# MOj0/vpt

Measured on AMD Instinct MI355X. Metric: volume samples/s, MCM 512^3 @ 1920x1080, higher is better.
Workload: dtype f32

## Files before the change

### vpt_amd/csrc/vpt_core.hip

```cpp
#include <chrono>
#include <memory>
#include "vpt_internal.h"
#include "vpt_kernels_layout.h"
#include "vpt_srgb_lut.h"

static thread_local char g_err[512] = "";
char *vpt_error_buffer(void) { return g_err; }
int fail(int code, const char *fmt, ...) {
    va_list ap; va_start(ap, fmt);
    vsnprintf(g_err, sizeof(g_err), fmt, ap);
    va_end(ap);
    return code;
}
extern "C" const char *vpt_last_error(void) { return g_err; }
extern "C" const char *vpt_version(void) { return "vpt-mi355x 0.1 (gfx950)"; }

extern "C" int vpt_device_count(int *count) {
    if (!count) return fail(VPT_ERR_INVALID, "count is null");
    HIP_TRY(hipGetDeviceCount(count));
    return VPT_OK;
}
extern "C" int vpt_context_create(int device, vpt_context **out) {
    if (!out) return fail(VPT_ERR_INVALID, "out is null");
    int n = 0;
// ... 940 lines not shown
static int profile_sum(const EventPairs &pairs, double *total_ms, uint32_t *launches) {
    double sum = 0.0; uint32_t n = 0;
    for (const EventPairs::Pair *p = pairs.first(); p; p = pairs.after(p)) {
        float ms = 0.0f;
        HIP_TRY(hipEventElapsedTime(&ms, p->t0, p->t1));
        sum += (double)ms; n += p->launches;
    }
    *total_ms = sum; *launches = n;
    return VPT_OK;
}
extern "C" int vpt_renderer_profile_side(vpt_renderer *r, double *total_ms, uint32_t *launches) {
    if (!r || !total_ms || !launches) return fail(VPT_ERR_INVALID, "null argument");
    HIP_TRY(hipSetDevice(r->ctx->device));
    VPT_TRY(join_side(r));
    HIP_TRY(hipStreamSynchronize(r->ctx->stream));
    return profile_sum(r->side_timing, total_ms, launches);
}
extern "C" int vpt_renderer_profile(vpt_renderer *r, double *total_ms, uint32_t *launches) {
    if (!r || !total_ms || !launches) return fail(VPT_ERR_INVALID, "null argument");
    HIP_TRY(hipSetDevice(r->ctx->device));
    HIP_TRY(hipStreamSynchronize(r->ctx->stream));
    return profile_sum(r->timing, total_ms, launches);
}

extern "C" int vpt_probe_math(vpt_context *c, int which, const float *in, float *out, size_t n) {
    if (!c || !in || !out) return fail(VPT_ERR_INVALID, "null argument");
    if (which < 0 || which > VPT_PROBE_POW) return fail(VPT_ERR_INVALID, "unknown probe %d", which);
    if (n == 0) return VPT_OK;
    HIP_TRY(hipSetDevice(c->device));
    size_t nin = (which == VPT_PROBE_ATAN2 || which == VPT_PROBE_MIN || which == VPT_PROBE_MAX || which == VPT_PROBE_POW) ? 2 * n : n;
    DevBuf<float> din, dout;
    HIP_TRY(din.alloc(nin));
    HIP_TRY(dout.alloc(n));
    HIP_TRY(hipMemcpyAsync(din, in, nin * sizeof(float), hipMemcpyHostToDevice, c->stream));
    hipLaunchKernelGGL(k_probe_math, dim3((unsigned)((n + 255) / 256)), dim3(256), 0, c->stream, which, din.get(), dout.get(), n);
    HIP_TRY(hipGetLastError());
    HIP_TRY(hipMemcpyAsync(out, dout, n * sizeof(float), hipMemcpyDeviceToHost, c->stream));
    HIP_TRY(hipStreamSynchronize(c->stream));
    return VPT_OK;
}
static int probe_sample(vpt_renderer *r, const float *xyz, float *rgba, size_t n, bool boundary) {
    if (!r || !xyz || !rgba) return fail(VPT_ERR_INVALID, "null argument");
    if (n == 0) return VPT_OK;
    vpt_context *c = r->ctx;
    HIP_TRY(hipSetDevice(c->device));
    PassArgs a;
    VPT_TRY(make_args(r, nullptr, true, &a));
    if (boundary && !a.vol.atlas) return fail(VPT_ERR_UNSUPPORTED, "the volume's boundary atlas is not in use (switched off, or a float volume with non-finite texels)");
    DevBuf<float> din; DevBuf<float4> dout;
    HIP_TRY(din.alloc(3 * n));
    HIP_TRY(dout.alloc(n));
    HIP_TRY(hipMemcpyAsync(din, xyz, 3 * n * sizeof(float), hipMemcpyHostToDevice, c->stream));
    dim3 grid((unsigned)((n + 255) / 256));
    const bool launched = dispatch_sampler_variant(variant_of(r), [&](auto V) {
        if (boundary) hipLaunchKernelGGL(k_probe_sample_boundary<V()>, grid, dim3(VPT_BLOCK), lds_bytes(r), c->stream, a, din.get(), dout.get(), n);
        else hipLaunchKernelGGL(k_probe_sample<V()>, grid, dim3(VPT_BLOCK), lds_bytes(r), c->stream, a, din.get(), dout.get(), n);
        return true;
    }, [] { return false; });
    if (!launched) return fail(VPT_ERR_INVALID, "no probe kernel for variant %d", variant_of(r));
    HIP_TRY(hipGetLastError());
    HIP_TRY(hipMemcpyAsync(rgba, dout, n * sizeof(float4), hipMemcpyDeviceToHost, c->stream));
    HIP_TRY(hipStreamSynchronize(c->stream));
    return VPT_OK;
}

extern "C" int vpt_probe_environment_texels(vpt_renderer *r, float *rgba, size_t n) {
    if (!r || !rgba) return fail(VPT_ERR_INVALID, "null argument");
    const size_t texels = (size_t)r->env_w * r->env_h;
    if (n < texels) return fail(VPT_ERR_INVALID, "environment table holds %zu texels, room for %zu", texels, n);
    vpt_context *c = r->ctx;
    HIP_TRY(hipSetDevice(c->device));
    VPT_TRY(join_side(r));
    HIP_TRY(hipMemcpyAsync(rgba, r->env, texels * sizeof(float4), hipMemcpyDeviceToHost, c->stream));
    HIP_TRY(hipStreamSynchronize(c->stream));
    return VPT_OK;
}
extern "C" int vpt_probe_sample(vpt_renderer *r, const float *xyz, float *rgba, size_t n) { return probe_sample(r, xyz, rgba, n, false); }
extern "C" int vpt_probe_sample_boundary(vpt_renderer *r, const float *xyz, float *rgba, size_t n) { return probe_sample(r, xyz, rgba, n, true); }

extern "C" int vpt_probe_stream_read(vpt_context *c, size_t nbytes, int iterations, double *gb_per_s) {
    if (!c || !gb_per_s) return fail(VPT_ERR_INVALID, "null argument");
    if (nbytes < (1u << 20) || iterations < 1) return fail(VPT_ERR_INVALID, "need at least 1 MiB and one iteration");
    HIP_TRY(hipSetDevice(c->device));
    size_t n16 = nbytes / 16;
    DevBuf<uint4> buf; DevBuf<uint32_t> sink;
    HIP_TRY(buf.alloc(n16));
    HIP_TRY(sink.alloc(1));
    HIP_TRY(hipMemsetAsync(buf, 0, n16 * 16, c->stream));
    Event e0, e1;
    float ms = 0.0f;
    HIP_TRY(e0.create());
    HIP_TRY(e1.create());
    dim3 grid(256 * 16);
    hipLaunchKernelGGL(k_stream_read, grid, dim3(VPT_BLOCK), 0, c->stream, buf.get(), n16, sink.get());
    HIP_TRY(hipEventRecord(e0, c->stream));
    for (int i = 0; i < iterations; i++) {
        hipLaunchKernelGGL(k_stream_read, grid, dim3(VPT_BLOCK), 0, c->stream, buf.get(), n16, sink.get());
        HIP_TRY(hipGetLastError());
    }
    HIP_TRY(hipEventRecord(e1, c->stream));
    HIP_TRY(hipEventSynchronize(e1));
    HIP_TRY(hipEventElapsedTime(&ms, e0, e1));
    *gb_per_s = (double)(n16 * 16) * iterations / ((double)ms * 1e-3) / 1e9;
    return VPT_OK;
}
```

### vpt_amd/csrc/vpt_device.h

```cpp
#pragma once
#include <hip/hip_runtime.h>
#include <stdint.h>
#include "vpt_variants.h"

#define VPT_DEV __device__ __forceinline__

struct f3 { float x, y, z; };
struct f2 { float x, y; };

VPT_DEV float vmin(float a, float b) { return fminf(a, b); }
VPT_DEV float vmax(float a, float b) { return fmaxf(a, b); }
VPT_DEV float vclamp01(float x) { return vmin(vmax(x, 0.0f), 1.0f); }
VPT_DEV float mixf(float a, float b, float t) { return fmaf(b, t, a * (1.0f - t)); }
VPT_DEV f3 mix3(f3 a, f3 b, float t) { return f3{ mixf(a.x, b.x, t), mixf(a.y, b.y, t), mixf(a.z, b.z, t) }; }
VPT_DEV float dot3(f3 a, f3 b) { return fmaf(a.z, b.z, fmaf(a.y, b.y, a.x * b.x)); }
VPT_DEV float length3(f3 a) { return sqrtf(dot3(a, a)); }
VPT_DEV f3 sub3(f3 a, f3 b) { return f3{ a.x - b.x, a.y - b.y, a.z - b.z }; }
VPT_DEV f3 madd3(f3 p, float t, f3 d) { return f3{ fmaf(t, d.x, p.x), fmaf(t, d.y, p.y), fmaf(t, d.z, p.z) }; }
VPT_DEV float lerpf(float a, float b, float f) { return fmaf(f, b - a, a); }
VPT_DEV float4 lerp4(float4 a, float4 b, float f) {
    return make_float4(lerpf(a.x, b.x, f), lerpf(a.y, b.y, f), lerpf(a.z, b.z, f), lerpf(a.w, b.w, f));
}

VPT_DEV float rcp_nr(float x) {
// ... 483 lines not shown
        uint32_t x, y, z; float fx, fy, fz;
        filter_cell<V>(p.x, v.fnx, v.hx, x, fx);
        filter_cell<V>(p.y, v.fny, v.hy, y, fy);
        filter_cell<V>(p.z, v.fnz, v.hz, z, fz);
        const float *b0 = (const float *)cell_addr<WIDE>(v, t, x, y, z);
        const bool lx = below_first(p.x, v.fnx), ly = below_first(p.y, v.fny), lz = below_first(p.z, v.fnz);
        f2 out = { 0.0f, 0.0f };
#pragma unroll
        for (int c = 0; c < (RG ? 2 : 1); c++) {
            const float *b = b0 + 128 * c;
            float2 r00, r10, r01, r11;
            __builtin_memcpy(&r00, b, 8); __builtin_memcpy(&r10, b + 5, 8); __builtin_memcpy(&r01, b + 25, 8); __builtin_memcpy(&r11, b + 30, 8);
            if (lx) { r00.y = r00.x; r10.y = r10.x; r01.y = r01.x; r11.y = r11.x; }
            if (ly) { r10 = r00; r11 = r01; }
            if (lz) { r01 = r00; r11 = r10; }
            float c00 = lerpf(r00.x, r00.y, fx), c10 = lerpf(r10.x, r10.y, fx);
            float c01 = lerpf(r01.x, r01.y, fx), c11 = lerpf(r11.x, r11.y, fx);
            const float val = lerpf(lerpf(c00, c10, fy), lerpf(c01, c11, fy), fz);
            if (c == 0) out.x = val; else out.y = val;
        }
        return out;
    }
    if (V & VPT_V_NEAREST) {
        uint32_t x = nearest_cell(p.x, v.fnx, v.hx), y = nearest_cell(p.y, v.fny, v.hy), z = nearest_cell(p.z, v.fnz, v.hz);
        const uint8_t *a = cell_addr<WIDE>(v, t, x, y, z);
        if (SNORM) return f2{ snorm_decode((float)(int8_t)a[0]), RG ? snorm_decode((float)(int8_t)a[128]) : 0.0f };
        return f2{ (float)a[0] * VPT_INV255, RG ? (float)a[128] * VPT_INV255 : 0.0f };
    }
    uint32_t x, y, z; float fx, fy, fz;
    filter_cell<V>(p.x, v.fnx, v.hx, x, fx);
    filter_cell<V>(p.y, v.fny, v.hy, y, fy);
    filter_cell<V>(p.z, v.fnz, v.hz, z, fz);
    if (V & VPT_V_REC) {
        const uint64_t w = record_load(record_addr<WIDE>(v, t, x, y, z));
        return f2{ record_blend((uint32_t)w, (uint32_t)(w >> 32), fx, fy, fz), 0.0f };
    }
    if ((V & VPT_V_ALIGNED) && !WIDE) {
        const uint32_t off = t.tx[x] + t.ty[y] + t.tz[z];
        return f2{ aligned_taps<SNORM>(v.bricks, off, fx, fy, fz), RG ? aligned_taps<SNORM>(v.bricks, off + 128u, fx, fy, fz) : 0.0f };
    }
    const uint8_t *a = cell_addr<WIDE>(v, t, x, y, z);
    return f2{ trilinear_taps<V>(a, fx, fy, fz), RG ? trilinear_taps<V>(a + 128, fx, fy, fz) : 0.0f };
}
template <int V>
VPT_DEV float sample_volume(const DevVolume &v, const LdsTables &t, f3 p) { return sample_volume_rg<V & ~VPT_V_RG>(v, t, p).x; }

VPT_DEV float4 sample_tf(const float4 *tf_pairs, float tf_fw, float tf_hi, float r) {
    float u = __builtin_amdgcn_fmed3f(fmaf(r, tf_fw, -0.5f), 0.0f, tf_hi);
    float f = __builtin_amdgcn_fractf(u);
    uint32_t i = (uint32_t)u;
    float4 a = tf_pairs[2 * i], d = tf_pairs[2 * i + 1];
    return make_float4(fmaf(f, d.x, a.x), fmaf(f, d.y, a.y), fmaf(f, d.z, a.z), fmaf(f, d.w, a.w));
}

struct DevEnv {
    const float4 *texels;
    int w, h;
    float4 constant;
};
VPT_DEV void linear_taps(float s, int n, int &i0, int &i1, float &f) {
    float fn = (float)n;
    float u = fmaf(s, fn, -0.5f);
    if (!(u > -1.0f)) u = -1.0f;
    if (u > fn) u = fn;
    float fl = floorf(u);
    f = u - fl;
    int i = (int)fl;
    i0 = min(max(i, 0), n - 1);
    i1 = min(max(i + 1, 0), n - 1);
}
VPT_DEV float4 sample_tf2d(const float4 *tf, int w, int h, float r, float g) {
    int x0, x1, y0, y1; float fx, fy;
    linear_taps(r, w, x0, x1, fx);
    linear_taps(g, h, y0, y1, fy);
    float4 r0 = lerp4(tf[(size_t)y0 * w + x0], tf[(size_t)y0 * w + x1], fx);
    float4 r1 = lerp4(tf[(size_t)y1 * w + x0], tf[(size_t)y1 * w + x1], fx);
    return lerp4(r0, r1, fy);
}
VPT_DEV float4 sample_environment(const DevEnv &e, f3 d) {
    if (e.w == 1 && e.h == 1) return e.constant;
    float a = vpt_atan2f(d.x, -d.z);
    float b = vpt_asinf(-d.y) * 2.0f;
    float s = fmaf(a * 0.31830988618f, 0.5f, 0.5f);
    float t = fmaf(b * 0.31830988618f, 0.5f, 0.5f);
    int x0, x1, y0, y1; float fx, fy;
    linear_taps(s, e.w, x0, x1, fx);
    linear_taps(t, e.h, y0, y1, fy);
    float4 r0 = lerp4(e.texels[(size_t)y0 * e.w + x0], e.texels[(size_t)y0 * e.w + x1], fx);
    float4 r1 = lerp4(e.texels[(size_t)y1 * e.w + x0], e.texels[(size_t)y1 * e.w + x1], fx);
    return lerp4(r0, r1, fy);
}
```

### vpt_amd/csrc/vpt_kernels.h

```cpp
#pragma once
#include "vpt_device.h"
#include "vpt_tonemap.h"

#define VPT_TILE        16
#define VPT_BLOCK       256
#define VPT_MAX_TRACK_ITERS 65536u
#ifndef VPT_UNROLL
#define VPT_UNROLL      4
#endif
#ifndef VPT_UNROLL_MIP
#define VPT_UNROLL_MIP  8
#endif
#define VPT_WAVES_ATTR(n)  VPT_WAVES_ATTR_(n)
#define VPT_WAVES_ATTR_(n) VPT_WAVES_ATTR_##n
#define VPT_WAVES_ATTR_0
#define VPT_WAVES_ATTR_2 __attribute__((amdgpu_waves_per_eu(2, 8)))
#define VPT_WAVES_ATTR_3 __attribute__((amdgpu_waves_per_eu(3, 8)))
#define VPT_WAVES_ATTR_4 __attribute__((amdgpu_waves_per_eu(4, 8)))
#define VPT_WAVES_ATTR_5 __attribute__((amdgpu_waves_per_eu(5, 8)))
#define VPT_WAVES_ATTR_6 __attribute__((amdgpu_waves_per_eu(6, 8)))
#define VPT_WAVES_ATTR_7 __attribute__((amdgpu_waves_per_eu(7, 8)))
#define VPT_WAVES_ATTR_8 __attribute__((amdgpu_waves_per_eu(8, 8)))
#ifndef VPT_MIP_WAVES
#define VPT_MIP_WAVES 6
// ... 14 lines not shown
#define VPT_DOS_WAVES 0
#endif

struct PixMap {
    int W, H;
    int local_h;
    int tiles_x, ntiles;
    int G, g, R;
    int rshift;
    int ty0;
    const float *ndc_x, *ndc_y;
    const uint32_t *tile_list;
    int list_n;
};
struct Pix { int i, j, l, k; bool valid, tile; };

VPT_DEV int global_row(const PixMap &m, int l) {
    if (m.G == 1) return l;
    int lb = (m.rshift >= 0) ? (l >> m.rshift) : (l / m.R);
    return (lb * m.G + m.g) * m.R + (l - lb * m.R);
}
VPT_DEV Pix map_pixel(const PixMap &m) {
    int xcd = (int)blockIdx.x & 7, ty = (int)blockIdx.y + m.ty0;
    int tx, w, lane = (int)threadIdx.x & 63;
    if (m.tile_list) {
        int e = (int)blockIdx.x;
        w = (int)threadIdx.x >> 6;
        if (blockDim.x == 64) {
            w = ((int)blockIdx.x >> 3) & 3;
            e = ((int)blockIdx.x >> 5) * 8 + xcd;
        }
        if (e >= m.list_n) { Pix q; q.i = q.j = q.l = q.k = 0; q.valid = false; q.tile = false; return q; }
        const uint32_t t = m.tile_list[e];
        tx = (int)(t & 0xffffu); ty = (int)(t >> 16);
    } else if (blockDim.x == 64) {
        w = ((int)blockIdx.x >> 3) & 3;
        tx = ((int)blockIdx.x >> 5) * 8 + ((xcd - ty) & 7);
    } else {
        w = (int)threadIdx.x >> 6;
        tx = ((int)blockIdx.x & ~7) + ((xcd - ty) & 7);
    }
    int t = ty * m.tiles_x + tx;
    Pix p;
    p.i = tx * VPT_TILE + (w & 1) * 8 + (lane & 7);
    p.l = ty * VPT_TILE + (w >> 1) * 8 + (lane >> 3);
    p.k = t * VPT_BLOCK + w * 64 + lane;
    p.j = global_row(m, p.l);
    p.valid = (p.i < m.W) && (p.l < m.local_h) && (p.j < m.H);
    p.tile = tx < m.tiles_x;
    return p;
}
VPT_DEV float ndc_col(const PixMap &m, int i) { return m.ndc_x[i]; }
VPT_DEV float ndc_row(const PixMap &m, int j) { return m.ndc_y[j]; }

struct LaoParams {
    int local_ambient_occlusion; float lao_weight; int num_lao_samples; float lao_step_size;
    int soft_shadows; float shadows_weight; int num_shadow_samples; float light_radius; float light_coefficient;
    float light_position[3];
};
struct DosParams { const float2 *samples; int nsamples; float scale_x, scale_y, depth; int tile_x0, tile_y0; };
struct PassArgs {
    PixMap pm;
    DevVolume vol;
    DevEnv env;
    const float4 *tf; int tf_w, tf_h; float tf_fw, tf_hi;
    Mat4 mvp_inv;
    float seed, offset, step, extinction, inv_extinction, anisotropy;
    uint32_t max_bounces, steps;
    f3 light;
    float mix, blur, inv_w, inv_h;
    float isovalue, gradient_step, threshold;
    union {
        LaoParams lao;
        DosParams dos;
    };
    uint32_t multi_passes;
    uint32_t miss_load_pos;
    uint32_t miss_verify;
    unsigned long long *violations;
    void *frame;
    void *acc;
    float4 *st0, *st1, *st2, *st3;
    uint2 *render;
    unsigned long long *samples;
    const struct FrameVar *frame_table;
    const uint8_t *tm_table;
    uint32_t frame_mask;
    uint32_t frame_base;
};
#define VPT_BUCKET_FRAMES 16
struct FrameVar { float seed, offset, mix, pad0; float lx, ly, lz, pad1; };
VPT_DEV uint32_t multi_pass_count(const PassArgs &a) { return a.multi_passes > 1u ? a.multi_passes : 1u; }
VPT_DEV void frame_select(PassArgs &a, uint32_t f) {
    if (a.frame_table) {
        FrameVar v = a.frame_table[(a.frame_base + f) & a.frame_mask];
        a.seed = v.seed; a.offset = v.offset; a.mix = v.mix;
        a.light = f3{ v.lx, v.ly, v.lz };
    }
}

template <bool WIDE, bool REC = false>
VPT_DEV LdsTables stage_lds(float4 *lds, const PassArgs &a) {
    const int nthreads = (int)blockDim.x;
    for (int t = (int)threadIdx.x; t < a.tf_w; t += nthreads) {
        float4 v = a.tf[t], n = a.tf[min(t + 1, a.tf_w - 1)];
        lds[2 * t] = v;
        lds[2 * t + 1] = make_float4(n.x - v.x, n.y - v.y, n.z - v.z, n.w - v.w);
    }
    int ntab = REC ? a.vol.nx + a.vol.ny : a.vol.nx + a.vol.ny + a.vol.nz;
    uint32_t *tab = (uint32_t *)(lds + 2 * a.tf_w);
    const uint32_t *src = REC ? (WIDE ? a.vol.rtabc : a.vol.rtab32) : (WIDE ? a.vol.tabc : a.vol.tab32);
    const int n4 = ntab >> 2;
    for (int t = (int)threadIdx.x; t < n4; t += nthreads) ((uint4 *)tab)[t] = ((const uint4 *)src)[t];
    for (int t = (n4 << 2) + (int)threadIdx.x; t < ntab; t += nthreads) tab[t] = src[t];
    __syncthreads();
    LdsTables r;
    r.tf = lds;
    r.tx = tab; r.ty = tab + a.vol.nx; r.tz = tab + (a.vol.nx + a.vol.ny);
    return r;
}
template <int V>
VPT_DEV float4 sample_volume_color(const PassArgs &a, const LdsTables &t, f3 p) {
    if (V & VPT_V_RG) {
        f2 rg = sample_volume_rg<V>(a.vol, t, p);
        return sample_tf2d(a.tf, a.tf_w, a.tf_h, rg.x, rg.y);
    }
    float r = sample_volume<V>(a.vol, t, p);
    return sample_tf(t.tf, a.tf_fw, a.tf_hi, r);
}
#define VPT_COUNTER_SLOTS 64
#define VPT_COUNTER_STRIDE 16
VPT_DEV void count_samples(unsigned long long *ctr, uint32_t n) {
    __shared__ uint32_t block_sum;
    if (threadIdx.x == 0) block_sum = 0;
    __syncthreads();
    for (int off = 32; off > 0; off >>= 1) n += __shfl_down(n, off);
    if (((int)threadIdx.x & 63) == 0 && n) atomicAdd(&block_sum, n);
    __syncthreads();
    if (threadIdx.x == 0 && block_sum)
        atomicAdd(ctr + (size_t)((blockIdx.y * gridDim.x + blockIdx.x) % VPT_COUNTER_SLOTS) * VPT_COUNTER_STRIDE, (unsigned long long)block_sum);
}
VPT_DEV uint2 pack_half4(float x, float y, float z, float w) {
    uint2 r;
    r.x = (uint32_t)to_half_bits(x) | ((uint32_t)to_half_bits(y) << 16);
    r.y = (uint32_t)to_half_bits(z) | ((uint32_t)to_half_bits(w) << 16);
    return r;
}
VPT_DEV void store_frame_texel(uint2 *dst, uint2 v) {
    __builtin_nontemporal_store(((unsigned long long)v.y << 32) | v.x, (unsigned long long *)dst);
}
VPT_DEV uint32_t tone_map_texel(const uint8_t *table, uint2 v, uint32_t **out) {
    typedef const TmFuse __attribute__((address_space(4))) *FuseArgs;
    const FuseArgs f = (FuseArgs)(uintptr_t)(table + VPT_TM_FUSE_OFFSET);
    const int mode = f->mode;
    if (out) *out = f->out;
    uint32_t rgb = (uint32_t)table[v.x & 0xffffu] | ((uint32_t)table[v.x >> 16] << 8) | ((uint32_t)table[v.y & 0xffffu] << 16);
    if (mode == 3) {
        const float low = f->low, range = f->range;
        float4 c = half4_to_float4(v);
        f3 w = { (c.x - low) / range, (c.y - low) / range, (c.z - low) / range };
        const float gray = 0.57735026918962576f;
        float z = (dot3(w, f3{ gray, gray, gray }) * gray) * f->one_minus_saturation;
        return ((z == 0.0f) ? rgb : 0u) | 0xff000000u;
    }
    return rgb | ((uint32_t)table[mode == 2 ? (v.y >> 16) : 65536u] << 24);
}
VPT_DEV void store_frame(const PassArgs &a, const Pix &p, uint2 v) {
    const size_t idx = (size_t)p.l * a.pm.W + p.i;
    store_frame_texel(&a.render[idx], v);
    if (a.tm_table) {
        uint32_t *out;
        const uint32_t texel = tone_map_texel(a.tm_table, v, &out);
        out[idx] = texel;
// ... 8 lines not shown
```

### vpt_amd/csrc/vpt_kernels_layout.h

```cpp
#pragma once
#include "vpt_kernels.h"


__global__ void __launch_bounds__(VPT_BLOCK) k_detile(PixMap pm, const uint8_t *src, uint8_t *dst, int elem) {
    Pix p = map_pixel(pm);
    if (!(p.i < pm.W && p.l < pm.local_h)) return;
    const uint8_t *s = src + (size_t)p.k * elem;
    uint8_t *d = dst + ((size_t)p.l * pm.W + p.i) * elem;
    for (int b = 0; b < elem; b++) d[b] = s[b];
}

__global__ void __launch_bounds__(VPT_BLOCK) k_detile_mcm3(PixMap pm, const f3 *src, float4 *dst) {
    Pix p = map_pixel(pm);
    if (!(p.i < pm.W && p.l < pm.local_h)) return;
    f3 v = src[p.k];
    dst[(size_t)p.l * pm.W + p.i] = make_float4(v.x, v.y, v.z, 0.0f);
}

__global__ void k_blit_block(uint8_t *vol, int nx, int ny, const uint8_t *blk, int x0, int y0, int z0, int bw, int bh, int bd, int ch) {
    size_t n = (size_t)bw * bh * bd;
    for (size_t t = (size_t)blockIdx.x * blockDim.x + threadIdx.x; t < n; t += (size_t)gridDim.x * blockDim.x) {
        int x = (int)(t % bw); size_t r = t / bw; int y = (int)(r % bh); int z = (int)(r / bh);
        size_t dst = (((size_t)(z0 + z) * ny + (y0 + y)) * nx + (x0 + x)) * ch;
        for (int c = 0; c < ch; c++) vol[dst + c] = blk[t * ch + c];
// ... 241 lines not shown
        }
}
__global__ void __launch_bounds__(256) k_scan_finite(const float *lin, size_t n, uint32_t *bad) {
    uint32_t b = 0;
    for (size_t i = (size_t)blockIdx.x * 256 + threadIdx.x; i < n; i += (size_t)gridDim.x * 256) b |= !(fabsf(lin[i]) < 1e37f);
    if (__builtin_amdgcn_ballot_w64(b != 0) && ((int)threadIdx.x & 63) == 0) atomicOr(bad, 1u);
}

typedef unsigned int vpt_u32x4 __attribute__((ext_vector_type(4)));
__global__ __launch_bounds__(VPT_BLOCK) void k_stream_read(const uint4 *src_, size_t n16, uint32_t *sink) {
    const vpt_u32x4 *src = (const vpt_u32x4 *)src_;
    size_t stride = (size_t)gridDim.x * VPT_BLOCK;
    vpt_u32x4 acc = { 0u, 0u, 0u, 0u };
    size_t i = (size_t)blockIdx.x * VPT_BLOCK + threadIdx.x;
    for (; i + 3 * stride < n16; i += 4 * stride) {
        vpt_u32x4 a = __builtin_nontemporal_load(src + i), b = __builtin_nontemporal_load(src + i + stride);
        vpt_u32x4 c = __builtin_nontemporal_load(src + i + 2 * stride), d = __builtin_nontemporal_load(src + i + 3 * stride);
        acc ^= a ^ b ^ c ^ d;
    }
    for (; i < n16; i += stride) acc ^= src[i];
    uint32_t v = acc.x ^ acc.y ^ acc.z ^ acc.w;
    if (v == 0x9E3779B9u) *sink = v;
}

__global__ void k_probe_math(int which, const float *in, float *out, size_t n) {
    size_t t = (size_t)blockIdx.x * blockDim.x + threadIdx.x;
    if (t >= n) return;
    float r = 0.0f, s, c;
    switch (which) {
        case 0: r = vpt_logf(in[t]); break;
        case 1: vpt_sincosf(in[t], s, c); r = s; break;
        case 2: vpt_sincosf(in[t], s, c); r = c; break;
        case 3: r = vpt_asinf(in[t]); break;
        case 4: r = vpt_atan2f(in[2 * t], in[2 * t + 1]); break;
        case 5: r = __uint_as_float(pcg(__float_as_uint(in[t]))); break;
        case 6: { uint32_t st = __float_as_uint(in[t]); r = random_uniform(st); } break;
        case 7: r = __uint_as_float((uint32_t)to_half_bits(in[t])); break;
        case 8: r = rcp_nr(in[t]); break;
        case 9: r = rsqrt_nr(in[t]); break;
        case 10: r = vmin(in[2 * t], in[2 * t + 1]); break;
        case 11: r = vmax(in[2 * t], in[2 * t + 1]); break;
        case 12: r = vpt_logf_uniform(in[t]); break;
        case 13: r = rcp_nrz(in[t]); break;
        case 14: r = sqrt_nr(in[t]); break;
        case 15: r = vpt_expf(in[t]); break;
        case 16: r = vpt_powf(in[2 * t], in[2 * t + 1]); break;
    }
    out[t] = r;
}
template <int V>
__global__ void __launch_bounds__(VPT_BLOCK) k_probe_sample_boundary(PassArgs a, const float *xyz, float4 *out, size_t n) {
    extern __shared__ float4 lds_raw[];
    LdsTables t = stage_lds<(V & VPT_V_WIDE) != 0>(lds_raw, a);
    size_t i = (size_t)blockIdx.x * blockDim.x + threadIdx.x;
    if (i >= n) return;
    const f3 q = { xyz[3 * i], xyz[3 * i + 1], xyz[3 * i + 2] };
    const bool oob = (vmax(vmax(q.x, q.y), q.z) > 1.0f) || (vmin(vmin(q.x, q.y), q.z) < 0.0f);
    if (!oob) { out[i] = sample_volume_color<V>(a, t, q); return; }
    constexpr bool PLAIN = !(V & (VPT_V_NEAREST | VPT_V_RG | VPT_V_F32 | VPT_V_SNORM | VPT_V_QCUBIC | VPT_V_NORM16));
    const f2 rg = PLAIN ? f2{ sample_volume_boundary(a.vol, q), 0.0f } : sample_boundary_rg<V>(a.vol, q);
    out[i] = (V & VPT_V_RG) ? sample_tf2d(a.tf, a.tf_w, a.tf_h, rg.x, rg.y) : sample_tf(t.tf, a.tf_fw, a.tf_hi, rg.x);
}
template <int V>
__global__ void __launch_bounds__(VPT_BLOCK) k_probe_sample(PassArgs a, const float *xyz, float4 *out, size_t n) {
    extern __shared__ float4 lds_raw[];
    LdsTables t = stage_lds<(V & VPT_V_WIDE) != 0>(lds_raw, a);
    size_t i = (size_t)blockIdx.x * blockDim.x + threadIdx.x;
    if (i >= n) return;
    out[i] = sample_volume_color<V>(a, t, f3{ xyz[3 * i], xyz[3 * i + 1], xyz[3 * i + 2] });
}
```

### vpt_amd/csrc/vpt_kernels_mcm.h

```cpp
#pragma once
#include "vpt_kernels.h"

struct Photon {
    f3 position, direction, transmittance, radiance;
    uint32_t bounces, samples;
};
template <bool NOBLUR = false>
VPT_DEV void unproject_rand(uint32_t &state, float px, float py, const PassArgs &a, f3 from0, f3 &from, f3 &to) {
    if (NOBLUR || a.blur == 0.0f) {
        random_uniform(state); random_uniform(state);
        from = from0;
    } else {
        f2 d = random_disk(state);
        from = dehomogenize(mat4_mul_point(a.mvp_inv, px + d.x * a.blur, py + d.y * a.blur, -1.0f));
    }
    float sx = random_uniform(state), sy = random_uniform(state);
    float ax = fmaf(sx, 2.0f, -1.0f) * a.inv_w;
    float ay = fmaf(sy, 2.0f, -1.0f) * a.inv_h;
    to = dehomogenize(mat4_mul_point(a.mvp_inv, px + ax, py + ay, 1.0f));
}
VPT_DEV f3 unproject_near(float px, float py, const PassArgs &a) {
    return dehomogenize(mat4_mul_point(a.mvp_inv, px + 0.0f, py + 0.0f, -1.0f));
}
VPT_DEV f3 photon_start(f3 from, f3 dir) {
// ... 433 lines not shown
    else mcm_events<V>(a, t, ph, px, py EV_ARG);
    photon_store(a, p.k, ph);
    if (FUSE_RENDER) store_frame(a, p, pack_half4(ph.radiance.x, ph.radiance.y, ph.radiance.z, 1.0f));
#ifdef VPT_EVENT_TIMING
    EV_MARK(evc, 6, "s_waitcnt vmcnt(0)");
    ev_flush(evc, a.violations);
#endif
}
template <bool FUSE_RENDER, int V>
__global__ void __launch_bounds__(VPT_BLOCK) __attribute__((amdgpu_waves_per_eu(5, 8))) k_mcm_integrate_early(PassArgs a) {
    frame_select(a, 0);
    Pix p = map_pixel(a.pm);
    PhotonState st;
    if (p.tile) st = photon_load(a, p.k);
    extern __shared__ float4 lds_raw[];
    LdsTables t = stage_lds<(V & VPT_V_WIDE) != 0, (V & VPT_V_REC) != 0>(lds_raw, a);
    if (!p.valid) return;
    float px = ndc_col(a.pm, p.i), py = ndc_row(a.pm, p.j);
    Photon ph = photon_unpack(st);
    if (V & VPT_V_FAST) mcm_events_fast_early<V & ~VPT_V_FAST>(a, t, ph, px, py);
    else mcm_events_early<V>(a, t, ph, px, py);
    photon_store(a, p.k, ph);
    if (FUSE_RENDER) store_frame(a, p, pack_half4(ph.radiance.x, ph.radiance.y, ph.radiance.z, 1.0f));
}
VPT_DEV const float4 *stage_tf_fill(float4 *lds, const PassArgs &a) {
    const int nthreads = (int)blockDim.x;
    for (int t = (int)threadIdx.x; t < a.tf_w; t += nthreads) {
        float4 v = a.tf[t], n = a.tf[min(t + 1, a.tf_w - 1)];
        lds[2 * t] = v;
        lds[2 * t + 1] = make_float4(n.x - v.x, n.y - v.y, n.z - v.z, n.w - v.w);
    }
    return lds;
}
VPT_DEV const float4 *stage_tf(float4 *lds, const PassArgs &a) {
    stage_tf_fill(lds, a);
    __syncthreads();
    return lds;
}
struct MissLoad { uint32_t aw; float fa, fb; };
template <bool CHECK>
VPT_DEV MissLoad miss_sample_issue(const PassArgs &a, f3 q, unsigned long long *violations) {
    MissLoad l;
    l.aw = atlas_dword(a.vol.atlas, boundary_cell(a.vol, q, l.fa, l.fb));
    if (CHECK) {
        const bool oob = (vmax(vmax(q.x, q.y), q.z) > 1.0f) || (vmin(vmin(q.x, q.y), q.z) < 0.0f);
        if (!oob) atomicAdd(violations, 1ull);
    }
    return l;
}
VPT_DEV void miss_sample_finish(const PassArgs &a, const float4 *tf, const MissLoad &l) {
    float4 vs = sample_tf(tf, a.tf_fw, a.tf_hi, boundary_blend(l.aw, l.fa, l.fb));
    asm volatile("" : "+v"(vs.w));
}
template <int V>
VPT_DEV void miss_sample_any(const PassArgs &a, const float4 *tf, f3 q) {
    const f2 rg = sample_boundary_rg<V>(a.vol, q);
    float4 vs = (V & VPT_V_RG) ? sample_tf2d(a.tf, a.tf_w, a.tf_h, rg.x, rg.y) : sample_tf(tf, a.tf_fw, a.tf_hi, rg.x);
    asm volatile("" : "+v"(vs.w));
    if (a.miss_verify) {
        const bool oob = (vmax(vmax(q.x, q.y), q.z) > 1.0f) || (vmin(vmin(q.x, q.y), q.z) < 0.0f);
        if (!oob) atomicAdd(a.violations, 1ull);
    }
}
VPT_DEV uint32_t pass_seed(float px, float py, float seed) {
    return hash3(__float_as_uint(ndc_to_uv(px)), __float_as_uint(ndc_to_uv(py)), __float_as_uint(seed));
}
template <int V, bool CHECK, bool LATE, bool DEPOSIT = true>
VPT_DEV void mcm_events_miss(const PassArgs &a, const float4 *tf, Photon &ph, float px, float py, f3 from0, uint32_t state) {
    for (uint32_t s = 0u; s < a.steps; s++) {
        float dist = random_exponential(state, a.inv_extinction);
        ph.position = madd3(ph.position, dist, ph.direction);
        constexpr bool OTHER = (V & (VPT_V_NEAREST | VPT_V_RG | VPT_V_F32 | VPT_V_SNORM)) != 0;
        MissLoad l = { 0u, 0.0f, 0.0f };
        if (OTHER) miss_sample_any<V>(a, tf, ph.position);
        else l = miss_sample_issue<CHECK>(a, ph.position, a.violations);
        if (!LATE && !OTHER) miss_sample_finish(a, tf, l);
        random_uniform(state);
        if (DEPOSIT) {
            float4 env = sample_environment(a.env, ph.direction);
            photon_deposit(ph, f3{ env.x, env.y, env.z });
        }
        reset_photon<true>(state, ph, px, py, a, from0);
        if (LATE && !OTHER) miss_sample_finish(a, tf, l);
    }
}
template <int V, bool CHECK, bool LATE, bool DEPOSIT = true>
VPT_DEV void mcm_events_miss_fast(const PassArgs &a, const float4 *tf, const FastPixel &c, Photon &ph, float px, float py, uint32_t state) {
    const float ld = fast_log2_scale(a.inv_extinction), ld32 = -32.0f * ld;
    for (uint32_t s = 0u; s < a.steps; s++) {
        float dist = fmaf(hw_log2(pcg_float(state)), ld, ld32);
        ph.position = madd3(ph.position, dist, ph.direction);
        constexpr bool OTHER = (V & (VPT_V_NEAREST | VPT_V_RG | VPT_V_F32 | VPT_V_SNORM)) != 0;
        MissLoad l = { 0u, 0.0f, 0.0f };
        if (OTHER) miss_sample_any<V>(a, tf, ph.position);
        else l = miss_sample_issue<CHECK>(a, ph.position, a.violations);
        if (!LATE && !OTHER) miss_sample_finish(a, tf, l);
        state = pcg(state);
        f3 rad = { 0.0f, 0.0f, 0.0f };
        if (DEPOSIT) { float4 env = sample_environment(a.env, ph.direction); rad = f3{ env.x, env.y, env.z }; }
        fast_path_end<true, DEPOSIT>(a, c, state, ph, rad, px, py);
        if (LATE && !OTHER) miss_sample_finish(a, tf, l);
    }
}
struct MissPixel { FastPixel c; f3 from0; uint32_t state; };
template <bool FAST>
VPT_DEV MissPixel miss_pixel_start(const PassArgs &a, float px, float py, float4 s1, f3 s0, Photon &ph) {
    MissPixel m;
    ph.direction = f3{ s1.x, s1.y, s1.z };
    ph.bounces = 0u;
    ph.transmittance = f3{ 1.0f, 1.0f, 1.0f };
    if (FAST) {
        m.c = fast_pixel(a, px, py);
        m.from0 = m.c.from0;
        ph.position = a.miss_load_pos ? s0 : photon_start_fast(m.c.from0, ph.direction);
    } else {
        m.from0 = unproject_near(px, py, a);
        ph.position = a.miss_load_pos ? s0 : photon_start(m.from0, ph.direction);
    }
    m.state = pass_seed(px, py, a.seed);
    asm volatile("" : "+v"(ph.position.x), "+v"(ph.position.y), "+v"(ph.position.z), "+v"(m.state));
    return m;
}
#ifdef VPT_EVENT_TIMING
#define EV_MISS_MARK(evc, slot, WAIT) EV_MARK(evc, slot, WAIT)
#define EV_MISS_PIN(x) asm volatile("" : "+v"(x))
#define EV_MISS_BEGIN(evc, ph) do { EV_PIN3((ph).position); EV_MARK(evc, 5, "s_waitcnt vmcnt(0) lgkmcnt(0)"); } while (0)
#define EV_MISS_EVENTS(evc, ph) do { EV_PIN3((ph).direction); EV_MARK(evc, 0, "s_waitcnt vmcnt(0) lgkmcnt(0)"); } while (0)
#define EV_MISS_END(evc, a) do { EV_MARK(evc, 6, "s_waitcnt vmcnt(0)"); ev_flush(evc, CHECK ? nullptr : (a).violations, VPT_TIMING_MISS_WAVES); } while (0)
#else
#define EV_MISS_MARK(evc, slot, WAIT) do { } while (0)
#define EV_MISS_PIN(x) do { } while (0)
#define EV_MISS_BEGIN(evc, ph) do { } while (0)
#define EV_MISS_EVENTS(evc, ph) do { } while (0)
#define EV_MISS_END(evc, a) do { } while (0)
#endif
template <bool FUSE_RENDER, int V, bool CHECK, bool LATE>
__global__ void __launch_bounds__(VPT_BLOCK)
__attribute__((amdgpu_waves_per_eu(((V & (VPT_V_NEAREST | VPT_V_RG | VPT_V_F32 | VPT_V_SNORM)) && !(V & VPT_V_FAST)) ? 7 : 8, 8))) k_mcm_miss(PassArgs a) {
    EV_LOCAL
    frame_select(a, 0);
    Pix p = map_pixel(a.pm);
    EV_MISS_PIN(p.k); EV_MISS_MARK(evc, 1, "s_waitcnt lgkmcnt(0)");
    float4 s1 = make_float4(0.0f, 0.0f, 1.0f, 0.0f), s3 = make_float4(0.0f, 0.0f, 0.0f, 0.0f);
    f3 s0 = { 0.0f, 0.0f, 0.0f };
    float px = 0.0f, py = 0.0f;
    if (p.tile) {
        s1 = a.st1[p.k]; s3 = a.st3[p.k];
        if (a.miss_load_pos) s0 = ((const f3 *)a.st0)[p.k];
    }
    if (p.valid) { px = ndc_col(a.pm, p.i); py = ndc_row(a.pm, p.j); }
    extern __shared__ float4 lds_raw[];
    const float4 *tf = stage_tf_fill(lds_raw, a);
    EV_MISS_MARK(evc, 2, "s_waitcnt vmcnt(0)");
    Photon ph;
    const MissPixel m = miss_pixel_start<(V & VPT_V_FAST) != 0>(a, px, py, s1, s0, ph);
    EV_MISS_MARK(evc, 3, "");
    __syncthreads();
    EV_MISS_MARK(evc, 4, "");
    if (!p.valid) return;
    ph.radiance = f3{ s3.x, s3.y, s3.z };
    ph.samples = (uint32_t)(s3.w + 0.5f);
    EV_MISS_BEGIN(evc, ph);
    if (V & VPT_V_FAST) mcm_events_miss_fast<V & ~VPT_V_FAST, CHECK, LATE>(a, tf, m.c, ph, px, py, m.state);
    else mcm_events_miss<V, CHECK, LATE>(a, tf, ph, px, py, m.from0, m.state);
    EV_MISS_EVENTS(evc, ph);
    a.st1[p.k] = make_float4(ph.direction.x, ph.direction.y, ph.direction.z, 0.0f);
    a.st3[p.k] = make_float4(ph.radiance.x, ph.radiance.y, ph.radiance.z, (float)ph.samples);
    if (FUSE_RENDER) store_frame(a, p, pack_half4(ph.radiance.x, ph.radiance.y, ph.radiance.z, 1.0f));
    EV_MISS_END(evc, a);
}
template <int V, bool CHECK, bool LATE>
__global__ void __launch_bounds__(VPT_BLOCK) __attribute__((amdgpu_waves_per_eu(8, 8))) k_mcm_miss_settled(PassArgs a) {
    EV_LOCAL
    frame_select(a, 0);
    Pix p = map_pixel(a.pm);
    EV_MISS_PIN(p.k); EV_MISS_MARK(evc, 1, "s_waitcnt lgkmcnt(0)");
    float4 s1 = make_float4(0.0f, 0.0f, 1.0f, 0.0f);
    f3 s0 = { 0.0f, 0.0f, 0.0f };
    float px = 0.0f, py = 0.0f;
    if (p.tile) {
        s1 = a.st1[p.k];
        if (a.miss_load_pos) s0 = ((const f3 *)a.st0)[p.k];
    }
    if (p.valid) { px = ndc_col(a.pm, p.i); py = ndc_row(a.pm, p.j); }
    extern __shared__ float4 lds_raw[];
    const float4 *tf = stage_tf_fill(lds_raw, a);
    EV_MISS_MARK(evc, 2, "s_waitcnt vmcnt(0)");
    Photon ph;
    const MissPixel m = miss_pixel_start<(V & VPT_V_FAST) != 0>(a, px, py, s1, s0, ph);
    EV_MISS_MARK(evc, 3, "");
    __syncthreads();
    EV_MISS_MARK(evc, 4, "");
    if (!p.valid) return;
    ph.radiance = f3{ 0.0f, 0.0f, 0.0f };
    ph.samples = 0u;
    EV_MISS_BEGIN(evc, ph);
    if (V & VPT_V_FAST) mcm_events_miss_fast<V & ~VPT_V_FAST, CHECK, LATE, false>(a, tf, m.c, ph, px, py, m.state);
    else mcm_events_miss<V, CHECK, LATE, false>(a, tf, ph, px, py, m.from0, m.state);
    EV_MISS_EVENTS(evc, ph);
    a.st1[p.k] = make_float4(ph.direction.x, ph.direction.y, ph.direction.z, 0.0f);
    EV_MISS_END(evc, a);
}
template <bool FAST>
__global__ void __launch_bounds__(VPT_BLOCK) k_mcm_materialize(PassArgs a, uint32_t pending) {
    Pix p = map_pixel(a.pm);
    if (!p.valid) return;
    if (pending) a.st3[p.k].w = (float)((uint32_t)(a.st3[p.k].w + 0.5f) + pending);
    const float px = ndc_col(a.pm, p.i), py = ndc_row(a.pm, p.j);
    const float4 s1 = a.st1[p.k];
    const f3 dir = { s1.x, s1.y, s1.z };
    f3 pos;
    if (FAST) pos = photon_start_fast(fast_pixel(a, px, py).from0, dir);
    else pos = photon_start(unproject_near(px, py, a), dir);
    ((f3 *)a.st0)[p.k] = pos;
    ((f3 *)a.st2)[p.k] = f3{ 1.0f, 1.0f, 1.0f };
}

template <int V, bool FRAMES>
VPT_DEV void mcm_multi_body(PassArgs &a, uint32_t npasses, uint2 *ring, uint32_t slot_pixels) {
    extern __shared__ float4 lds_raw[];
    LdsTables t = stage_lds<(V & VPT_V_WIDE) != 0, (V & VPT_V_REC) != 0>(lds_raw, a);
    Pix p = map_pixel(a.pm);
    if (!p.valid) return;
    float px = ndc_col(a.pm, p.i), py = ndc_row(a.pm, p.j);
    Photon ph = photon_unpack(photon_load(a, p.k));
    for (uint32_t f = 0; f < npasses; f++) {
        a.seed = a.frame_table[(a.frame_base + f) & a.frame_mask].seed;
        EV_LOCAL
        if (V & VPT_V_FAST) mcm_events_fast<V & ~VPT_V_FAST>(a, t, ph, px, py EV_ARG);
        else mcm_events<V>(a, t, ph, px, py EV_ARG);
        if (FRAMES) store_frame_texel(&ring[(size_t)f * slot_pixels + (size_t)p.l * a.pm.W + p.i], pack_half4(ph.radiance.x, ph.radiance.y, ph.radiance.z, 1.0f));
    }
    photon_store(a, p.k, ph);
    store_frame_texel(&a.render[(size_t)p.l * a.pm.W + p.i], pack_half4(ph.radiance.x, ph.radiance.y, ph.radiance.z, 1.0f));
}
template <int V>
__global__ void __launch_bounds__(VPT_BLOCK) __attribute__((amdgpu_waves_per_eu(VPT_MULTI_WAVES, 8))) k_mcm_multi(PassArgs a, uint32_t npasses) {
    mcm_multi_body<V, false>(a, npasses, nullptr, 0u);
}
template <int V>
__global__ void __launch_bounds__(VPT_BLOCK) __attribute__((amdgpu_waves_per_eu(4, 8))) k_mcm_frames(PassArgs a, uint32_t npasses, uint2 *ring, uint32_t slot_pixels) {
    mcm_multi_body<V, true>(a, npasses, ring, slot_pixels);
}

struct FrameSeeds { float seed[VPT_BUCKET_FRAMES]; };
template <bool DISPLAY>
VPT_DEV void bucket_store(const PassArgs &a, void *ring, size_t texel, uint2 v) {
    if (DISPLAY) ((uint32_t *)ring)[texel] = tone_map_texel(a.tm_table, v, nullptr);
    else store_frame_texel((uint2 *)ring + texel, v);
}
template <int V, bool EARLY, bool DISPLAY>
__global__ void __launch_bounds__(VPT_BLOCK) __attribute__((amdgpu_waves_per_eu(4, 8)))
k_mcm_bucket_hit(PassArgs a, FrameSeeds fs, uint32_t nframes, void *ring, uint32_t slot_pixels) {
// ... 77 lines not shown
```

Baseline: 231.0 billion.

## Drive miss kernels from a tile list with per-wave alpha-only TF staging

```diff
diff --git a/vpt_amd/csrc/vpt_core.hip b/vpt_amd/csrc/vpt_core.hip
--- a/vpt_amd/csrc/vpt_core.hip
+++ b/vpt_amd/csrc/vpt_core.hip
@@ -1016,12 +1016,20 @@
     HIP_TRY(dout.alloc(n));
     HIP_TRY(hipMemcpyAsync(din, xyz, 3 * n * sizeof(float), hipMemcpyHostToDevice, c->stream));
     dim3 grid((unsigned)((n + 255) / 256));
+    const size_t lds = boundary ? lds_bytes(r) + 4 + (size_t)r->tf_w * 32 : lds_bytes(r);
+    int prepared = VPT_OK;
     const bool launched = dispatch_sampler_variant(variant_of(r), [&](auto V) {
-        if (boundary) hipLaunchKernelGGL(k_probe_sample_boundary<V()>, grid, dim3(VPT_BLOCK), lds_bytes(r), c->stream, a, din.get(), dout.get(), n);
-        else hipLaunchKernelGGL(k_probe_sample<V()>, grid, dim3(VPT_BLOCK), lds_bytes(r), c->stream, a, din.get(), dout.get(), n);
+        if (boundary) {
+            prepared = lds_prepare((const void *)k_probe_sample_boundary<V()>, lds);
+            if (prepared == VPT_OK) hipLaunchKernelGGL(k_probe_sample_boundary<V()>, grid, dim3(VPT_BLOCK), lds, c->stream, a, din.get(), dout.get(), n);
+        } else {
+            prepared = lds_prepare((const void *)k_probe_sample<V()>, lds);
+            if (prepared == VPT_OK) hipLaunchKernelGGL(k_probe_sample<V()>, grid, dim3(VPT_BLOCK), lds, c->stream, a, din.get(), dout.get(), n);
+        }
         return true;
     }, [] { return false; });
     if (!launched) return fail(VPT_ERR_INVALID, "no probe kernel for variant %d", variant_of(r));
+    VPT_TRY(prepared);
     HIP_TRY(hipGetLastError());
     HIP_TRY(hipMemcpyAsync(rgba, dout, n * sizeof(float4), hipMemcpyDeviceToHost, c->stream));
     HIP_TRY(hipStreamSynchronize(c->stream));
diff --git a/vpt_amd/csrc/vpt_device.h b/vpt_amd/csrc/vpt_device.h
--- a/vpt_amd/csrc/vpt_device.h
+++ b/vpt_amd/csrc/vpt_device.h
@@ -559,6 +559,13 @@
     float4 a = tf_pairs[2 * i], d = tf_pairs[2 * i + 1];
     return make_float4(fmaf(f, d.x, a.x), fmaf(f, d.y, a.y), fmaf(f, d.z, a.z), fmaf(f, d.w, a.w));
 }
+VPT_DEV float sample_tf_alpha(const float2 *alpha_pairs, float tf_fw, float tf_hi, float r) {
+    float u = __builtin_amdgcn_fmed3f(fmaf(r, tf_fw, -0.5f), 0.0f, tf_hi);
+    float f = __builtin_amdgcn_fractf(u);
+    uint32_t i = (uint32_t)u;
+    float2 p = alpha_pairs[i];
+    return fmaf(f, p.y, p.x);
+}
 
 struct DevEnv {
     const float4 *texels;
diff --git a/vpt_amd/csrc/vpt_kernels.h b/vpt_amd/csrc/vpt_kernels.h
--- a/vpt_amd/csrc/vpt_kernels.h
+++ b/vpt_amd/csrc/vpt_kernels.h
@@ -90,6 +90,18 @@
 }
 VPT_DEV float ndc_col(const PixMap &m, int i) { return m.ndc_x[i]; }
 VPT_DEV float ndc_row(const PixMap &m, int j) { return m.ndc_y[j]; }
+VPT_DEV Pix map_listed_pixel(const PixMap &m, uint32_t t) {
+    const int tx = (int)(t & 0xffffu), ty = (int)(t >> 16);
+    const int w = (int)threadIdx.x >> 6, lane = (int)threadIdx.x & 63;
+    Pix p;
+    p.i = tx * VPT_TILE + (w & 1) * 8 + (lane & 7);
+    p.l = ty * VPT_TILE + (w >> 1) * 8 + (lane >> 3);
+    p.k = (ty * m.tiles_x + tx) * VPT_BLOCK + w * 64 + lane;
+    p.j = global_row(m, p.l);
+    p.valid = (p.i < m.W) && (p.l < m.local_h) && (p.j < m.H);
+    p.tile = tx < m.tiles_x;
+    return p;
+}
 
 struct LaoParams {
     int local_ambient_occlusion; float lao_weight; int num_lao_samples; float lao_step_size;
@@ -157,6 +169,19 @@
     r.tx = tab; r.ty = tab + a.vol.nx; r.tz = tab + (a.vol.nx + a.vol.ny);
     return r;
 }
+struct TfAlpha { float w, n; };
+VPT_DEV float2 *tf_alpha_column(void *lds, int tf_w) { return (float2 *)lds + ((int)threadIdx.x >> 6) * tf_w; }
+VPT_DEV TfAlpha tf_alpha_load(const float4 *tf, int tf_w, int t) { return TfAlpha{ tf[t].w, tf[min(t + 1, tf_w - 1)].w }; }
+VPT_DEV void tf_alpha_store(float2 *col, int t, TfAlpha v) { col[t] = make_float2(v.w, v.n - v.w); }
+VPT_DEV void tf_alpha_fence() {
+    __builtin_amdgcn_fence(__ATOMIC_RELEASE, "wavefront");
+    __builtin_amdgcn_wave_barrier();
+    __builtin_amdgcn_fence(__ATOMIC_ACQUIRE, "wavefront");
+}
+VPT_DEV void tf_alpha_stage_rest(float2 *col, const float4 *tf, int tf_w) {
+#pragma unroll 1
+    for (int t = ((int)threadIdx.x & 63) + 64; t < tf_w; t += 64) tf_alpha_store(col, t, tf_alpha_load(tf, tf_w, t));
+}
 template <int V>
 VPT_DEV float4 sample_volume_color(const PassArgs &a, const LdsTables &t, f3 p) {
     if (V & VPT_V_RG) {
diff --git a/vpt_amd/csrc/vpt_kernels_layout.h b/vpt_amd/csrc/vpt_kernels_layout.h
--- a/vpt_amd/csrc/vpt_kernels_layout.h
+++ b/vpt_amd/csrc/vpt_kernels_layout.h
@@ -317,14 +317,25 @@
 __global__ void __launch_bounds__(VPT_BLOCK) k_probe_sample_boundary(PassArgs a, const float *xyz, float4 *out, size_t n) {
     extern __shared__ float4 lds_raw[];
     LdsTables t = stage_lds<(V & VPT_V_WIDE) != 0>(lds_raw, a);
+    constexpr bool PLAIN = !(V & (VPT_V_NEAREST | VPT_V_RG | VPT_V_F32 | VPT_V_SNORM | VPT_V_QCUBIC | VPT_V_NORM16));
+    float2 *col = nullptr;
+    if (PLAIN) {
+        const int ntab = a.vol.nx + a.vol.ny + a.vol.nz;
+        col = tf_alpha_column((float2 *)lds_raw + 4 * a.tf_w + ((ntab + 1) >> 1), a.tf_w);
+        const int lane = (int)threadIdx.x & 63;
+        if (lane < a.tf_w) tf_alpha_store(col, lane, tf_alpha_load(a.tf, a.tf_w, lane));
+        tf_alpha_stage_rest(col, a.tf, a.tf_w);
+        tf_alpha_fence();
+    }
     size_t i = (size_t)blockIdx.x * blockDim.x + threadIdx.x;
     if (i >= n) return;
     const f3 q = { xyz[3 * i], xyz[3 * i + 1], xyz[3 * i + 2] };
     const bool oob = (vmax(vmax(q.x, q.y), q.z) > 1.0f) || (vmin(vmin(q.x, q.y), q.z) < 0.0f);
     if (!oob) { out[i] = sample_volume_color<V>(a, t, q); return; }
-    constexpr bool PLAIN = !(V & (VPT_V_NEAREST | VPT_V_RG | VPT_V_F32 | VPT_V_SNORM | VPT_V_QCUBIC | VPT_V_NORM16));
     const f2 rg = PLAIN ? f2{ sample_volume_boundary(a.vol, q), 0.0f } : sample_boundary_rg<V>(a.vol, q);
-    out[i] = (V & VPT_V_RG) ? sample_tf2d(a.tf, a.tf_w, a.tf_h, rg.x, rg.y) : sample_tf(t.tf, a.tf_fw, a.tf_hi, rg.x);
+    float4 c = (V & VPT_V_RG) ? sample_tf2d(a.tf, a.tf_w, a.tf_h, rg.x, rg.y) : sample_tf(t.tf, a.tf_fw, a.tf_hi, rg.x);
+    if (PLAIN) c.w = sample_tf_alpha(col, a.tf_fw, a.tf_hi, rg.x);
+    out[i] = c;
 }
 template <int V>
 __global__ void __launch_bounds__(VPT_BLOCK) k_probe_sample(PassArgs a, const float *xyz, float4 *out, size_t n) {
diff --git a/vpt_amd/csrc/vpt_kernels_mcm.h b/vpt_amd/csrc/vpt_kernels_mcm.h
--- a/vpt_amd/csrc/vpt_kernels_mcm.h
+++ b/vpt_amd/csrc/vpt_kernels_mcm.h
@@ -509,6 +509,10 @@
     float4 vs = sample_tf(tf, a.tf_fw, a.tf_hi, boundary_blend(l.aw, l.fa, l.fb));
     asm volatile("" : "+v"(vs.w));
 }
+VPT_DEV void miss_sample_finish(const PassArgs &a, const float2 *tf_alpha, const MissLoad &l) {
+    float w = sample_tf_alpha(tf_alpha, a.tf_fw, a.tf_hi, boundary_blend(l.aw, l.fa, l.fb));
+    asm volatile("" : "+v"(w));
+}
 template <int V>
 VPT_DEV void miss_sample_any(const PassArgs &a, const float4 *tf, f3 q) {
     const f2 rg = sample_boundary_rg<V>(a.vol, q);
@@ -522,41 +526,41 @@
 VPT_DEV uint32_t pass_seed(float px, float py, float seed) {
     return hash3(__float_as_uint(ndc_to_uv(px)), __float_as_uint(ndc_to_uv(py)), __float_as_uint(seed));
 }
-template <int V, bool CHECK, bool LATE, bool DEPOSIT = true>
-VPT_DEV void mcm_events_miss(const PassArgs &a, const float4 *tf, Photon &ph, float px, float py, f3 from0, uint32_t state) {
+template <int V, bool CHECK, bool LATE, bool DEPOSIT = true, typename TF>
+VPT_DEV void mcm_events_miss(const PassArgs &a, TF tf, Photon &ph, float px, float py, f3 from0, uint32_t state) {
     for (uint32_t s = 0u; s < a.steps; s++) {
         float dist = random_exponential(state, a.inv_extinction);
         ph.position = madd3(ph.position, dist, ph.direction);
         constexpr bool OTHER = (V & (VPT_V_NEAREST | VPT_V_RG | VPT_V_F32 | VPT_V_SNORM)) != 0;
         MissLoad l = { 0u, 0.0f, 0.0f };
-        if (OTHER) miss_sample_any<V>(a, tf, ph.position);
+        if constexpr (OTHER) miss_sample_any<V>(a, tf, ph.position);
         else l = miss_sample_issue<CHECK>(a, ph.position, a.violations);
-        if (!LATE && !OTHER) miss_sample_finish(a, tf, l);
+        if constexpr (!LATE && !OTHER) miss_sample_finish(a, tf, l);
         random_uniform(state);
         if (DEPOSIT) {
             float4 env = sample_environment(a.env, ph.direction);
             photon_deposit(ph, f3{ env.x, env.y, env.z });
         }
         reset_photon<true>(state, ph, px, py, a, from0);
-        if (LATE && !OTHER) miss_sample_finish(a, tf, l);
-    }
-}
-template <int V, bool CHECK, bool LATE, bool DEPOSIT = true>
-VPT_DEV void mcm_events_miss_fast(const PassArgs &a, const float4 *tf, const FastPixel &c, Photon &ph, float px, float py, uint32_t state) {
+        if constexpr (LATE && !OTHER) miss_sample_finish(a, tf, l);
+    }
+}
+template <int V, bool CHECK, bool LATE, bool DEPOSIT = true, typename TF>
+VPT_DEV void mcm_events_miss_fast(const PassArgs &a, TF tf, const FastPixel &c, Photon &ph, float px, float py, uint32_t state) {
     const float ld = fast_log2_scale(a.inv_extinction), ld32 = -32.0f * ld;
     for (uint32_t s = 0u; s < a.steps; s++) {
         float dist = fmaf(hw_log2(pcg_float(state)), ld, ld32);
         ph.position = madd3(ph.position, dist, ph.direction);
         constexpr bool OTHER = (V & (VPT_V_NEAREST | VPT_V_RG | VPT_V_F32 | VPT_V_SNORM)) != 0;
         MissLoad l = { 0u, 0.0f, 0.0f };
-        if (OTHER) miss_sample_any<V>(a, tf, ph.position);
+        if constexpr (OTHER) miss_sample_any<V>(a, tf, ph.position);
         else l = miss_sample_issue<CHECK>(a, ph.position, a.violations);
-        if (!LATE && !OTHER) miss_sample_finish(a, tf, l);
+        if constexpr (!LATE && !OTHER) miss_sample_finish(a, tf, l);
         state = pcg(state);
         f3 rad = { 0.0f, 0.0f, 0.0f };
         if (DEPOSIT) { float4 env = sample_environment(a.env, ph.direction); rad = f3{ env.x, env.y, env.z }; }
         fast_path_end<true, DEPOSIT>(a, c, state, ph, rad, px, py);
-        if (LATE && !OTHER) miss_sample_finish(a, tf, l);
+        if constexpr (LATE && !OTHER) miss_sample_finish(a, tf, l);
     }
 }
 struct MissPixel { FastPixel c; f3 from0; uint32_t state; };
@@ -591,10 +595,74 @@
 #define EV_MISS_EVENTS(evc, ph) do { } while (0)
 #define EV_MISS_END(evc, a) do { } while (0)
 #endif
+struct MissWave { Pix p; float px, py; const float2 *tf_alpha; MissPixel m; float4 s3; };
+template <bool FAST, bool RADIANCE>
+VPT_DEV bool miss_wave_start(PassArgs &a, void *lds, MissWave &w, Photon &ph EV_PARAM) {
+    const int e = (int)blockIdx.x;
+    if (e >= a.pm.list_n) return false;
+    const uint32_t entry = a.pm.tile_list[e];
+    frame_select(a, 0);
+    w.p = map_listed_pixel(a.pm, entry);
+    const Pix &p = w.p;
+    if (__ballot(p.valid) == 0ull) return false;
+    EV_MISS_PIN(w.p.k); EV_MISS_MARK(evc, 1, "s_waitcnt lgkmcnt(0)");
+    float px = 0.0f, py = 0.0f;
+    if (p.valid) { px = ndc_col(a.pm, p.i); py = ndc_row(a.pm, p.j); }
+    const int lane = (int)threadIdx.x & 63, tf_w = a.tf_w;
+    float2 *const col = tf_alpha_column(lds, tf_w);
+    TfAlpha c0 = { 0.0f, 0.0f };
+    if (lane < tf_w) c0 = tf_alpha_load(a.tf, tf_w, lane);
+    asm volatile("" ::: "memory");
+    float4 s1 = a.st1[p.k];
+    f3 s0;
+    if (a.miss_load_pos) s0 = ((const f3 *)a.st0)[p.k];
+    w.s3 = make_float4(0.0f, 0.0f, 0.0f, 0.0f);
+    if (RADIANCE) w.s3 = a.st3[p.k];
+    asm volatile("" ::: "memory");
+    EV_MISS_PIN(px); EV_MISS_PIN(py); EV_MISS_MARK(evc, 2, "");
+    MissPixel &m = w.m;
+    if (FAST) m.c = fast_pixel(a, px, py);
+    else m.c.from0 = unproject_near(px, py, a);
+    m.state = pass_seed(px, py, a.seed);
+    if (lane < tf_w) tf_alpha_store(col, lane, c0);
+    if (FAST) asm volatile("" : "+v"(m.c.fb.x), "+v"(m.c.fb.y), "+v"(m.c.fb.z), "+v"(m.c.fb.w));
+    asm volatile("" : "+v"(m.c.from0.x), "+v"(m.c.from0.y), "+v"(m.c.from0.z), "+v"(m.state) : : "memory");
+    EV_MISS_MARK(evc, 3, "");
+    asm volatile("" : "+v"(s1.x), "+v"(s1.y), "+v"(s1.z), "+v"(m.c.from0.x), "+v"(m.c.from0.y), "+v"(m.c.from0.z), "+v"(m.state));
+    EV_MISS_MARK(evc, 4, "");
+    if (tf_w > 64) tf_alpha_stage_rest(col, a.tf, tf_w);
+    tf_alpha_fence();
+    m.from0 = m.c.from0;
+    ph.direction = f3{ s1.x, s1.y, s1.z };
+    ph.bounces = 0u;
+    ph.transmittance = f3{ 1.0f, 1.0f, 1.0f };
+    if (FAST) ph.position = a.miss_load_pos ? s0 : photon_start_fast(m.from0, ph.direction);
+    else ph.position = a.miss_load_pos ? s0 : photon_start(m.from0, ph.direction);
+    w.px = px; w.py = py; w.tf_alpha = col;
+    return p.valid;
+}
 template <bool FUSE_RENDER, int V, bool CHECK, bool LATE>
 __global__ void __launch_bounds__(VPT_BLOCK)
 __attribute__((amdgpu_waves_per_eu(((V & (VPT_V_NEAREST | VPT_V_RG | VPT_V_F32 | VPT_V_SNORM)) && !(V & VPT_V_FAST)) ? 7 : 8, 8))) k_mcm_miss(PassArgs a) {
     EV_LOCAL
+    if constexpr (!(V & (VPT_V_NEAREST | VPT_V_RG | VPT_V_F32 | VPT_V_SNORM))) {
+        extern __shared__ float4 lds_raw[];
+        MissWave w;
+        Photon ph;
+        if (!miss_wave_start<(V & VPT_V_FAST) != 0, true>(a, lds_raw, w, ph EV_ARG)) return;
+        const Pix &p = w.p;
+        ph.radiance = f3{ w.s3.x, w.s3.y, w.s3.z };
+        ph.samples = (uint32_t)(w.s3.w + 0.5f);
+        EV_MISS_BEGIN(evc, ph);
+        if (V & VPT_V_FAST) mcm_events_miss_fast<V & ~VPT_V_FAST, CHECK, LATE>(a, w.tf_alpha, w.m.c, ph, w.px, w.py, w.m.state);
+        else mcm_events_miss<V, CHECK, LATE>(a, w.tf_alpha, ph, w.px, w.py, w.m.from0, w.m.state);
+        EV_MISS_EVENTS(evc, ph);
+        a.st1[p.k] = make_float4(ph.direction.x, ph.direction.y, ph.direction.z, 0.0f);
+        a.st3[p.k] = make_float4(ph.radiance.x, ph.radiance.y, ph.radiance.z, (float)ph.samples);
+        if (FUSE_RENDER) store_frame(a, p, pack_half4(ph.radiance.x, ph.radiance.y, ph.radiance.z, 1.0f));
+        EV_MISS_END(evc, a);
+        return;
+    }
     frame_select(a, 0);
     Pix p = map_pixel(a.pm);
     EV_MISS_PIN(p.k); EV_MISS_MARK(evc, 1, "s_waitcnt lgkmcnt(0)");
@@ -629,33 +697,17 @@
 template <int V, bool CHECK, bool LATE>
 __global__ void __launch_bounds__(VPT_BLOCK) __attribute__((amdgpu_waves_per_eu(8, 8))) k_mcm_miss_settled(PassArgs a) {
     EV_LOCAL
-    frame_select(a, 0);
-    Pix p = map_pixel(a.pm);
-    EV_MISS_PIN(p.k); EV_MISS_MARK(evc, 1, "s_waitcnt lgkmcnt(0)");
-    float4 s1 = make_float4(0.0f, 0.0f, 1.0f, 0.0f);
-    f3 s0 = { 0.0f, 0.0f, 0.0f };
-    float px = 0.0f, py = 0.0f;
-    if (p.tile) {
-        s1 = a.st1[p.k];
-        if (a.miss_load_pos) s0 = ((const f3 *)a.st0)[p.k];
-    }
-    if (p.valid) { px = ndc_col(a.pm, p.i); py = ndc_row(a.pm, p.j); }
     extern __shared__ float4 lds_raw[];
-    const float4 *tf = stage_tf_fill(lds_raw, a);
-    EV_MISS_MARK(evc, 2, "s_waitcnt vmcnt(0)");
+    MissWave w;
     Photon ph;
-    const MissPixel m = miss_pixel_start<(V & VPT_V_FAST) != 0>(a, px, py, s1, s0, ph);
-    EV_MISS_MARK(evc, 3, "");
-    __syncthreads();
-    EV_MISS_MARK(evc, 4, "");
-    if (!p.valid) return;
+    if (!miss_wave_start<(V & VPT_V_FAST) != 0, false>(a, lds_raw, w, ph EV_ARG)) return;
     ph.radiance = f3{ 0.0f, 0.0f, 0.0f };
     ph.samples = 0u;
     EV_MISS_BEGIN(evc, ph);
-    if (V & VPT_V_FAST) mcm_events_miss_fast<V & ~VPT_V_FAST, CHECK, LATE, false>(a, tf, m.c, ph, px, py, m.state);
-    else mcm_events_miss<V, CHECK, LATE, false>(a, tf, ph, px, py, m.from0, m.state);
+    if (V & VPT_V_FAST) mcm_events_miss_fast<V & ~VPT_V_FAST, CHECK, LATE, false>(a, w.tf_alpha, w.m.c, ph, w.px, w.py, w.m.state);
+    else mcm_events_miss<V, CHECK, LATE, false>(a, w.tf_alpha, ph, w.px, w.py, w.m.from0, w.m.state);
     EV_MISS_EVENTS(evc, ph);
-    a.st1[p.k] = make_float4(ph.direction.x, ph.direction.y, ph.direction.z, 0.0f);
+    a.st1[w.p.k] = make_float4(ph.direction.x, ph.direction.y, ph.direction.z, 0.0f);
     EV_MISS_END(evc, a);
 }
 template <bool FAST>
```

Measured after the change: 235.6 billion, median of 6. 2.0% higher.
